# tier4/icp_rust

Measured on AMD Instinct MI355X. Metric: ICP iterations/sec on 1M-pt 3D pair, higher is better.
Workload: dtype f64

## Files before the change

### icp_rust_amd/csrc/gn_win.hip

```cpp
#include "common.hpp"
#include "gn_device.hpp"
#include "gn_win_device.hpp"
#include "gn_loop.hpp"

namespace icp {


template <bool SUMS, int BATCH = kWinBatch>
__device__ __forceinline__ void win_hist_body(const double2 *__restrict__ a, const double2 *__restrict__ b,
                                              const Pose &T, double *__restrict__ rx, double *__restrict__ ry,
                                              unsigned n, const WinParams &P, uint32_t *whist, WinState *st,
                                              GnScalars *scal, double *partials, int status_cls = -1) {
  __shared__ uint32_t lh[2 * kWinBins];
  if (SUMS && status_cls >= 0 && blockIdx.x == 0 && threadIdx.x < (unsigned)kShardStatusWords)
    whist[2 * kWinBins + threadIdx.x] = (int)threadIdx.x == status_cls ? 1u : 0u;
  double acc[SUMS ? kNSum : 1];
#pragma unroll
  for (int k = 0; k < (SUMS ? kNSum : 1); ++k) acc[k] = 0.;
#ifdef ICP_WIN_DEBUG
  long long wst[6];
  wst[0] = wall_clock64();
#endif
  for (unsigned i = threadIdx.x; i < 2u * kWinBins; i += kWinThreads) lh[i] = 0;
  __syncthreads();
// ... 662 lines not shown
  np.T = outer;
  if (usable) {
    double acc[kNAcc], delta[3];
#pragma unroll
    for (int k = 0; k < kNAcc; ++k) acc[k] = combine_sum(s_tot, k, sig);
    if (solve_update(acc, acc + 9, delta) &&
        !((delta[0] * delta[0] + delta[1] * delta[1]) + delta[2] * delta[2] < ICP_DELTA_NORM_THRESHOLD)) {
      bool in_range;
      const Pose step = transform_new_in_range(delta, &in_range);
      if (in_range) {
        const Pose inner = transform_mul(step, transform_identity());
        np.T = transform_mul(inner, outer);
        np.valid = 1;
      }
    }
  }
  *ahead = np;
  res->next_pose = np.T;
  res->next_valid = np.valid;
}

static_assert(kWinThreads == kReduceThreads, "the launches of an evaluation share the reduction tree's geometry");
template <bool LISTS>
__global__ __launch_bounds__(kWinThreads) void k_win_finish(const double *__restrict__ rx,
                                                            const double *__restrict__ ry, unsigned n, WinParams P,
                                                            uint32_t *whist, WinState *st, double *wmed, double *wring,
                                                            GnScalars *scal, const double *partials, int sum_blocks,
                                                            SelCtl *ctl, GnResult *res, unsigned seq,
                                                            const unsigned *__restrict__ llen, unsigned lcap,
                                                            AheadPose *ahead, Pose outer) {
  constexpr int PM = kWinCapMed / kReduceThreads, PR = kWinCapRing / kReduceThreads;
  WinSel sel;
#ifdef ICP_WIN_DEBUG
  long long fst[10];
  fst[0] = wall_clock64();
#endif
  double *const totals = const_cast<double *>(partials) + (size_t)kTreeMaxBlocks * (kNSum + 1);
  const bool fold_early = gridDim.x >= (unsigned)(kNSum + 1) && sum_blocks <= kReduceMaxBlocks;
  const double fold_x = (fold_early && blockIdx.x < (unsigned)(kNSum + 1)) ? fold_one_load(partials, sum_blocks, (int)blockIdx.x) : 0.;
  bool fail = win_compact_body<LISTS, true>(rx, ry, n, n, P, whist, st, wmed, wring, llen, lcap, sel);
  if (fold_early && blockIdx.x < (unsigned)(kNSum + 1)) {
    __shared__ double s_fold4[4];
    const double tot = fold_one_reduce(fold_x, sum_blocks, s_fold4);
    if (threadIdx.x == 0) __hip_atomic_store(&totals[blockIdx.x], tot, __ATOMIC_RELAXED, __HIP_MEMORY_SCOPE_AGENT);
  }
#ifdef ICP_WIN_DEBUG
  fst[1] = wall_clock64();
#endif
  if (!last_block_arrives(&ctl->t[2])) return;
#ifdef ICP_WIN_DEBUG
  fst[2] = wall_clock64();
#endif
  const unsigned tid = threadIdx.x;
  double med[2] = {0., 0.}, sig[2] = {0., 0.};
  __shared__ double s_tot[kNSum + 1];
  const int nan_flag = __hip_atomic_load(&scal->nan_flag, __ATOMIC_RELAXED, __HIP_MEMORY_SCOPE_AGENT);
  {
    double vm[2][PM], vr[2][PR];
#pragma unroll
    for (int d = 0; d < 2; ++d) {
#pragma unroll
      for (int u = 0; u < PM; ++u)
        vm[d][u] = (fail || tid + u * kReduceThreads < sel.med_cnt[d])
                       ? __hip_atomic_load(&wmed[(size_t)d * kWinCapMed + tid + u * kReduceThreads], __ATOMIC_RELAXED,
                                           __HIP_MEMORY_SCOPE_AGENT)
                       : 0.;
#pragma unroll
      for (int u = 0; u < PR; ++u)
        vr[d][u] = (fail || tid + u * kReduceThreads < sel.ring_cnt[d])
                       ? __hip_atomic_load(&wring[(size_t)d * kWinCapRing + tid + u * kReduceThreads], __ATOMIC_RELAXED,
                                           __HIP_MEMORY_SCOPE_AGENT)
                       : 0.;
    }
    unsigned got[4];
#pragma unroll
    for (int k = 0; k < 4; ++k)
      got[k] = __hip_atomic_load(&st->list_cnt[k][0], __ATOMIC_RELAXED, __HIP_MEMORY_SCOPE_AGENT);
    if (fold_early) {
      if (tid < kNSum + 1) s_tot[tid] = __hip_atomic_load(&totals[tid], __ATOMIC_RELAXED, __HIP_MEMORY_SCOPE_AGENT);
    } else if (sum_blocks <= kReduceMaxBlocks) {
      fold_block_sums_256(partials, sum_blocks, s_tot);
    } else {
      fold_block_sums_lean(partials, sum_blocks, s_tot);
    }
    for (unsigned i = tid; i < 2u * kWinBins; i += kWinThreads)
      __hip_atomic_store(&whist[i], 0u, __ATOMIC_RELAXED, __HIP_MEMORY_SCOPE_AGENT);
    fail = fail || got[0] != sel.med_cnt[0] || got[1] != sel.med_cnt[1] || got[2] != sel.ring_cnt[0] ||
           got[3] != sel.ring_cnt[1];
    const unsigned klo = (n - 1) / 2, khi = n / 2;
    if (!fail) {
      unsigned long long key[2][2];
      const double m_lo[2] = {sel.range[0][0], sel.range[1][0]}, m_hi[2] = {sel.range[0][1], sel.range[1][1]};
      const long long mlo[2] = {(long long)klo - sel.med_base[0], (long long)klo - sel.med_base[1]};
      const long long mhi[2] = {(long long)khi - sel.med_base[0], (long long)khi - sel.med_base[1]};
#ifdef ICP_WIN_DEBUG
      fst[3] = wall_clock64();
#endif
      select_n<2, PM>(vm, sel.med_cnt, m_lo, m_hi, mlo, mhi, key, fail);
#ifdef ICP_WIN_DEBUG
      fst[4] = wall_clock64();
#endif
      if (!fail) {
#pragma unroll
        for (int d = 0; d < 2; ++d) {
          med[d] = middle_of(n, key[d][0], key[d][1]);
#pragma unroll
          for (int u = 0; u < PR; ++u) vr[d][u] = fabs(vr[d][u] - med[d]);
        }
        const double r_lo[2] = {sel.range[0][2], sel.range[1][2]}, r_hi[2] = {sel.range[0][3], sel.range[1][3]};
        const long long dlo[2] = {(long long)klo - sel.inner[0], (long long)klo - sel.inner[1]};
        const long long dhi[2] = {(long long)khi - sel.inner[0], (long long)khi - sel.inner[1]};
        select_n<2, PR>(vr, sel.ring_cnt, r_lo, r_hi, dlo, dhi, key, fail);
        if (!fail) {
          sig[0] = ICP_PPF34 * middle_of(n, key[0][0], key[0][1]);
          sig[1] = ICP_PPF34 * middle_of(n, key[1][0], key[1][1]);
        } else {
          med[0] = med[1] = 0.;
        }
      }
    }
  }
  if (tid == 0 && fail) st->fail = 1u;
  asm volatile("s_waitcnt vmcnt(0)" ::: "memory");
  __syncthreads();
  if (ahead && tid == 0) fill_ahead_pose(s_tot, sig, !fail && !nan_flag, outer, ahead, res);
#ifdef ICP_WIN_DEBUG
  fst[5] = wall_clock64();
#endif
  publish_folded(s_tot, res, seq, sig, med, nan_flag, fail ? 2 : 0);
#ifdef ICP_WIN_DEBUG
  asm volatile("s_waitcnt vmcnt(0)" ::: "memory");
  fst[6] = wall_clock64();
  if (tid == 0 && seq % 16 == 5)
    printf("[F last blk %d of %d] compact %lld ticket %lld loads %lld sel1 %lld sel2 %lld publish %lld (x10ns) cnt %u %u %u %u\n", blockIdx.x,
           gridDim.x, fst[1] - fst[0], fst[2] - fst[1], fst[3] - fst[2], fst[4] - fst[3], fst[5] - fst[4], fst[6] - fst[5],
           sel.med_cnt[0], sel.med_cnt[1], sel.ring_cnt[0], sel.ring_cnt[1]);
#endif
}

struct PickLds {
  union {
    struct {
      uint32_t cum[2 * kWinBins];
      uint32_t med[2][kWinCapMed], ring[2][kWinCapRing];
    } g;
    SelectLds<2> sel;
  };
};

struct PickDimLds {
  union {
    struct {
      uint32_t cum[kWinBins];
      uint32_t med[kWinCapMed], ring[kWinCapRing];
    } g;
    SelectLds<1> sel;
  };
};

struct WinBins1 {
  unsigned mlo, mhi, a0, b1, i0, i1;
  bool fail;
};
struct WinSel1 {
  unsigned med_base, med_cnt, inner, ring_cnt;
  double range[4];
};

__device__ __forceinline__ WinBins1 win_resolve_dim(const uint32_t *__restrict__ row, unsigned n, const WinDim &w,
                                                    WinState *st, int d, uint32_t *cum, WinSel1 &sel) {
  __shared__ unsigned s_wtot[kReduceThreads / 64];
  __shared__ int s_j[2], s_t[2], s_rng[7];
  __shared__ unsigned s_selu[4];
  __shared__ double s_seld[4];
  constexpr int PER = kWinBins / kReduceThreads, NW = kReduceThreads / 64;
  static_assert(PER == 4, "one 16-byte load per thread");
  const int tid = threadIdx.x, lane = tid & 63, wave = tid >> 6;
  const unsigned klo = (n - 1) / 2, khi = n / 2;
  if (tid < 2) s_j[tid] = -1;
  const uint4 x = reinterpret_cast<const uint4 *>(row)[tid];
  const unsigned v[PER] = {x.x, x.y, x.z, x.w};
  const unsigned tot = (x.x + x.y) + (x.z + x.w);
  const unsigned inc = wave_scan_inclusive(tot);
  if (lane == 63) s_wtot[wave] = inc;
  __syncthreads();
  {
    unsigned wbase = 0;
#pragma unroll
    for (int q = 0; q < NW; ++q) wbase += (q < wave) ? s_wtot[q] : 0u;
    unsigned run = wbase + inc - tot;
#pragma unroll
    for (int i = 0; i < PER; ++i) {
      cum[PER * tid + i] = run;
      if (run <= klo && klo < run + v[i]) s_j[0] = PER * tid + i;
      if (run <= khi && khi < run + v[i]) s_j[1] = PER * tid + i;
      run += v[i];
    }
  }
  __syncthreads();
  WinGeom geo = {};
  if (wave < 2) {
    geo = window_geometry(cum, n, w, s_j[0], s_j[1]);
    const int t = geo.ok ? bracket_search(cum, n, w, geo, wave) : -1;
    if (lane == 0) s_t[wave] = t;
  }
  __syncthreads();
  if (wave == 0) {
    WinRanges R = {};
    unsigned med_base = 0, med_cnt = 0, inner = 0, ring_cnt = 0;
    double range[4] = {0., 0., 0., 0.};
    unsigned counted = 0;
#pragma unroll
    for (int q = 0; q < NW; ++q) counted += s_wtot[q];
    bool ok = counted == n && resolve_window(cum, n, w, geo, s_t[0], s_t[1], R, med_base, med_cnt, inner, ring_cnt, range);
    if (ok)
      ok = R.mlo >= kF1 && R.mhi < kC1 && R.i0 <= R.i1 && R.a0 >= kF0 && R.i0 - 1 < kC0 && R.i1 + 1 >= kF2 &&
           R.b1 <= kWinBins - 2;
    if (lane == 0) {
      s_rng[0] = R.mlo;
      s_rng[1] = R.mhi;
      s_rng[2] = R.a0;
      s_rng[3] = R.b1;
      s_rng[4] = R.i0;
      s_rng[5] = R.i1;
      s_rng[6] = ok ? 0 : 1;
      s_selu[0] = med_base;
      s_selu[1] = med_cnt;
      s_selu[2] = inner;
      s_selu[3] = ring_cnt;
#pragma unroll
      for (int k = 0; k < 4; ++k) s_seld[k] = range[k];
      if (st) {
        st->med_base[d] = med_base;
        st->med_cnt[d] = med_cnt;
        st->ring_inner[d] = inner;
        st->ring_cnt[d] = ring_cnt;
        st->med_lo[d] = range[0];
        st->med_hi[d] = range[1];
        st->ring_lo[d] = range[2];
        st->ring_hi[d] = range[3];
      }
    }
  }
  __syncthreads();
  WinBins1 B;
  B.mlo = (unsigned)s_rng[0];
  B.mhi = (unsigned)s_rng[1];
  B.a0 = (unsigned)s_rng[2];
  B.b1 = (unsigned)s_rng[3];
  B.i0 = (unsigned)s_rng[4];
  B.i1 = (unsigned)s_rng[5];
  B.fail = s_rng[6] != 0;
  sel.med_base = s_selu[0];
  sel.med_cnt = s_selu[1];
  sel.inner = s_selu[2];
  sel.ring_cnt = s_selu[3];
#pragma unroll
  for (int k = 0; k < 4; ++k) sel.range[k] = s_seld[k];
  return B;
}

struct PickArgs {
  unsigned n;
  WinParams P;
  uint32_t *whist;
  WinState *st;
  const double *seg_all;
  const unsigned short *dir_all;
  int segments;
  GnScalars *scal;
  const double *partials;
  int sum_blocks;
  GnResult *res;
  unsigned seq;
  AheadPose *ahead;
  Pose outer;
  WinJoin *join;
};

__device__ __forceinline__ void win_pick_dim_body(const PickArgs &A, const int d, const bool primary, PickDimLds &L) {
  const unsigned n = A.n;
  WinState *const st = A.st;
  const double *__restrict__ seg_all = A.seg_all;
  const unsigned short *__restrict__ dir_all = A.dir_all;
  WinJoin *const J = A.join;
  constexpr int PM = kWinCapMed / kReduceThreads, PR = kWinCapRing / kReduceThreads;
  static_assert(kReduceMaxBlocks * 2 == kReduceThreads, "two threads per segment");
  static_assert(kBktStage <= (1 << 12), "descriptor: segment << 12 | position");
  __shared__ double s_tot[kNSum + 1];
  __shared__ unsigned s_cnt[2];
  __shared__ int s_last;
  __shared__ unsigned s_pflags;
  __shared__ double s_pms[2];
  const unsigned tid = threadIdx.x;
#ifdef ICP_WIN_DEBUG
  long long pst[10];
  pst[0] = wall_clock64();
  for (int k = 1; k < 10; ++k) pst[k] = pst[0];
#define PSTAMP(k) pst[k] = wall_clock64()
#else
#define PSTAMP(k)
#endif
  if (tid < 2) s_cnt[tid] = 0;
  const int nan_flag = __hip_atomic_load(&A.scal->nan_flag, __ATOMIC_RELAXED, __HIP_MEMORY_SCOPE_AGENT);
  const unsigned stage_overflow = __hip_atomic_load(&st->stage_overflow, __ATOMIC_RELAXED, __HIP_MEMORY_SCOPE_AGENT);
  WinSel1 sel;
  const WinBins1 R = win_resolve_dim(A.whist + (size_t)d * kWinBins, n, A.P.d[d], primary ? st : nullptr, d, L.g.cum, sel);
  double fx[kFoldQ];
  fold256_half_load(A.partials, A.sum_blocks, d, fx);
  PSTAMP(1);
  const bool fail = R.fail;
  bool bucket_miss = stage_overflow != 0, sel_fail = false;
  double med = 0., sig = 0.;
  {
    const bool usable = !fail && !bucket_miss;
    const unsigned w = tid & (unsigned)(kReduceMaxBlocks - 1), part = tid / (unsigned)kReduceMaxBlocks;
    if (usable && (int)w < A.segments) {
      const unsigned short *dir = dir_all + (size_t)w * kBktDir;
      if (part == 0) {
        const unsigned fm = word_to_fine(d, R.mlo), len_m = R.mhi - R.mlo + 1u;
        const unsigned m0 = dir[fm], m_end = dir[fm + len_m];
        const unsigned cm = m_end - m0;
        if (cm) {
          const unsigned pos = atomicAdd(&s_cnt[0], cm);
          for (unsigned k = 0; k < cm; ++k)
            if (pos + k < (unsigned)kWinCapMed) L.g.med[pos + k] = (w << 12) | (m0 + k);
        }
      } else {
        const unsigned fa = word_to_fine(d, R.a0), fb = word_to_fine(d, R.i1 + 1u);
        const unsigned len_a = R.i0 - R.a0, len_b = R.b1 - R.i1;
        const unsigned a_beg = dir[fa], a_end = dir[fa + len_a], b_beg = dir[fb], b_end = dir[fb + len_b];
        const unsigned cr = (a_end - a_beg) + (b_end - b_beg);
        if (cr) {
          unsigned pos = atomicAdd(&s_cnt[1], cr);
          for (unsigned k = a_beg; k < a_end; ++k, ++pos)
            if (pos < (unsigned)kWinCapRing) L.g.ring[pos] = (w << 12) | k;
          for (unsigned k = b_beg; k < b_end; ++k, ++pos)
            if (pos < (unsigned)kWinCapRing) L.g.ring[pos] = (w << 12) | k;
        }
      }
    }
    __syncthreads();
    PSTAMP(2);
    if (usable) bucket_miss = s_cnt[0] != sel.med_cnt || s_cnt[1] != sel.ring_cnt;
    const bool go = usable && !bucket_miss;
    double vm[1][PM], vr[1][PR];
#pragma unroll
    for (int u = 0; u < PM; ++u) {
      const unsigned e = tid + u * kReduceThreads;
      vm[0][u] = 0.;
      if (go && e < sel.med_cnt) {
        const uint32_t x = L.g.med[e];
        vm[0][u] = seg_all[(size_t)(x >> 12) * kBktStage + (x & 0xfffu)];
      }
    }
#pragma unroll
    for (int u = 0; u < PR; ++u) {
      const unsigned e = tid + u * kReduceThreads;
      vr[0][u] = 0.;
      if (go && e < sel.ring_cnt) {
        const uint32_t x = L.g.ring[e];
        vr[0][u] = seg_all[(size_t)(x >> 12) * kBktStage + (x & 0xfffu)];
      }
    }
    {
      unsigned long long *row = reinterpret_cast<unsigned long long *>(A.whist + (size_t)d * kWinBins);
#pragma unroll
      for (int u = 0; u < kWinBins / 2 / kReduceThreads; ++u)
        __hip_atomic_store(&row[tid + u * kReduceThreads], 0ull, __ATOMIC_RELAXED, __HIP_MEMORY_SCOPE_AGENT);
    }
    fold256_half_reduce(fx, A.sum_blocks, s_tot + d * kFoldH);
    __syncthreads();
    PSTAMP(3);
    const unsigned klo = (n - 1) / 2, khi = n / 2;
    if (go) {
      unsigned long long key[1][2];
      const unsigned cm[1] = {sel.med_cnt}, cr[1] = {sel.ring_cnt};
      const double m_lo[1] = {sel.range[0]}, m_hi[1] = {sel.range[1]};
      const long long mlo[1] = {(long long)klo - sel.med_base}, mhi[1] = {(long long)khi - sel.med_base};
      select_n_lds<1, PM>(vm, cm, m_lo, m_hi, mlo, mhi, key, sel_fail, L.sel);
      PSTAMP(4);
      if (!sel_fail) {
        med = middle_of(n, key[0][0], key[0][1]);
#pragma unroll
        for (int u = 0; u < PR; ++u) vr[0][u] = fabs(vr[0][u] - med);
        const double r_lo[1] = {sel.range[2]}, r_hi[1] = {sel.range[3]};
        const long long dlo[1] = {(long long)klo - sel.inner}, dhi[1] = {(long long)khi - sel.inner};
        select_n_lds<1, PR>(vr, cr, r_lo, r_hi, dlo, dhi, key, sel_fail, L.sel);
        PSTAMP(5);
        if (!sel_fail) sig = ICP_PPF34 * middle_of(n, key[0][0], key[0][1]);
      }
    }
  }
  const unsigned flags = (fail ? 1u : 0u) | (bucket_miss ? 2u : 0u) | (sel_fail ? 4u : 0u);
  WinJoinDim *const mine = &J->dim[d];
  if (tid < (unsigned)kFoldH) __hip_atomic_store(&mine->tot[tid], s_tot[d * kFoldH + tid], __ATOMIC_RELAXED, __HIP_MEMORY_SCOPE_AGENT);
  if (tid == 64) {
    __hip_atomic_store(&mine->med, med, __ATOMIC_RELAXED, __HIP_MEMORY_SCOPE_AGENT);
    __hip_atomic_store(&mine->sig, sig, __ATOMIC_RELAXED, __HIP_MEMORY_SCOPE_AGENT);
    __hip_atomic_store(&mine->flags, flags, __ATOMIC_RELAXED, __HIP_MEMORY_SCOPE_AGENT);
  }
  asm volatile("s_waitcnt vmcnt(0)" ::: "memory");
  __syncthreads();
  PSTAMP(6);
  if (tid == 0)
    s_last = (int)(__hip_atomic_fetch_add(&J->ticket, 1u, __ATOMIC_RELAXED, __HIP_MEMORY_SCOPE_AGENT) & 1u);
  __syncthreads();
  if (!s_last) {
#ifdef ICP_WIN_DEBUG
    if (tid == 0 && A.seq % 16 == 5)
      printf("[P%d first] resolve %lld list %lld load+fold %lld sel1 %lld sel2 %lld store %lld (x10ns) cnt %u %u\n", d,
             pst[1] - pst[0], pst[2] - pst[1], pst[3] - pst[2], pst[4] - pst[3], pst[5] - pst[4], pst[6] - pst[5],
             sel.med_cnt, sel.ring_cnt);
#endif
    return;
  }
  const int o = 1 - d;
  const WinJoinDim *const other = &J->dim[o];
  static_assert(offsetof(WinJoinDim, tot) == 16 && offsetof(WinJoinDim, flags) == 96, "words of the record");
  if (tid < 13) {
    const unsigned long long x =
        __hip_atomic_load(reinterpret_cast<const unsigned long long *>(other) + tid, __ATOMIC_RELAXED, __HIP_MEMORY_SCOPE_AGENT);
    if (tid < 2) s_pms[tid] = __longlong_as_double((long long)x);
    else if (tid < 12) s_tot[o * kFoldH + (tid - 2)] = __longlong_as_double((long long)x);
    else s_pflags = (unsigned)x;
  }
  __syncthreads();
  PSTAMP(7);
  const unsigned all = flags | s_pflags;
  const bool any_fail = (all & 1u) != 0, any_bucket = (all & 2u) != 0;
  const bool failed = any_fail || (!any_bucket && (all & 4u) != 0);
  const bool missed = failed || any_bucket;
  const double m_me = missed ? 0. : med, s_me = missed ? 0. : sig, m_ot = missed ? 0. : s_pms[0], s_ot = missed ? 0. : s_pms[1];
  const double med2[2] = {d ? m_ot : m_me, d ? m_me : m_ot}, sig2[2] = {d ? s_ot : s_me, d ? s_me : s_ot};
  if (tid == 0) {
    if (missed) st->fail = 1u;
    else if (primary) st->fail = 0u;
    if (stage_overflow) __hip_atomic_store(&st->stage_overflow, 0u, __ATOMIC_RELAXED, __HIP_MEMORY_SCOPE_AGENT);
  }
  const int overflow = missed ? (failed ? 2 : 3) : 0;
  GnResult *const res = A.res;
  if (A.ahead) {
    if (tid == 0) fill_ahead_pose(s_tot, sig2, !missed && !nan_flag, A.outer, A.ahead, res);
    publish_values<1>(s_tot, res, sig2, med2, nan_flag, overflow);
    PSTAMP(8);
    __syncthreads();
    publish_seq(res, A.seq);
  } else {
    PSTAMP(8);
    publish_folded(s_tot, res, A.seq, sig2, med2, nan_flag, overflow);
  }
#ifdef ICP_WIN_DEBUG
  asm volatile("s_waitcnt vmcnt(0)" ::: "memory");
  PSTAMP(9);
  if (tid == 0 && A.seq % 16 == 5)
    printf("[P%d last] resolve %lld list %lld load+fold %lld sel1 %lld sel2 %lld store %lld ticket+loads %lld ahead %lld "
           "publish %lld (x10ns) cnt %u %u\n", d, pst[1] - pst[0], pst[2] - pst[1], pst[3] - pst[2], pst[4] - pst[3],
           pst[5] - pst[4], pst[6] - pst[5], pst[7] - pst[6], pst[8] - pst[7], pst[9] - pst[8], sel.med_cnt, sel.ring_cnt);
#endif
#undef PSTAMP
}

__global__ __launch_bounds__(kReduceThreads) void k_win_pick(PickArgs A) {
  __shared__ PickDimLds L;
  win_pick_dim_body(A, (int)blockIdx.x, true, L);
}

__global__ __launch_bounds__(kWinThreads, 4) void k_win_hist_sums_bkt2(HistBktArgs A, HistBktArgs B) {
  __shared__ HistBktLds S;
  const unsigned half = gridDim.x >> 1;
  if (blockIdx.x < half) win_hist_sums_bkt_body(A, blockIdx.x, half, S);
  else win_hist_sums_bkt_body(B, blockIdx.x - half, half, S);
}
__global__ __launch_bounds__(kReduceThreads) void k_win_pick2(PickArgs A, PickArgs B) {
  __shared__ PickDimLds L;
  if (blockIdx.x < 2u) win_pick_dim_body(A, (int)blockIdx.x, true, L);
  else win_pick_dim_body(B, (int)blockIdx.x - 2, false, L);
}

namespace {
constexpr long long kPipeTimeoutTicks = 300000000;
__device__ __forceinline__ void pst_u32(unsigned *p, unsigned v) { __hip_atomic_store(p, v, __ATOMIC_RELAXED, __HIP_MEMORY_SCOPE_SYSTEM); }
__device__ __forceinline__ void pst_f64(double *p, double v) { __hip_atomic_store(p, v, __ATOMIC_RELAXED, __HIP_MEMORY_SCOPE_SYSTEM); }
__device__ __forceinline__ unsigned pld_u32(const unsigned *p) { return __hip_atomic_load(p, __ATOMIC_RELAXED, __HIP_MEMORY_SCOPE_SYSTEM); }
__device__ __forceinline__ double pld_f64(const double *p) { return __hip_atomic_load(p, __ATOMIC_RELAXED, __HIP_MEMORY_SCOPE_SYSTEM); }

__device__ __forceinline__ bool pipe_poll(const unsigned long long *words, int count, unsigned gen, LoopInbox *const *box, int W,
                                          LoopInbox *me, unsigned *payload_or) {
  __shared__ int s_pok;
  __shared__ unsigned s_ppay;
  if (threadIdx.x < 64) {
    const int lane = (int)threadIdx.x;
    unsigned long long seen = 0;
    int ok = 1;
    const long long t0 = wall_clock64();
    for (;;) {
      bool here = true;
      if (lane < count) {
        seen = __hip_atomic_load(&words[lane], __ATOMIC_RELAXED, __HIP_MEMORY_SCOPE_SYSTEM);
        here = (int)((unsigned)seen - gen) >= 0;
      }
      if (__all(here)) break;
      int stop = 0;
      if (lane == 0) {
        if (pld_u32(&me->abort[0]) != 0u) stop = 1;
        else if (wall_clock64() - t0 > kPipeTimeoutTicks) {
          for (int q = 0; q < W; ++q) pst_u32(&box[q]->abort[0], 1u);
          stop = 1;
        }
      }
      if (__builtin_amdgcn_readfirstlane(stop)) {
        ok = 0;
        break;
      }
      __builtin_amdgcn_s_sleep(1);
    }
    unsigned pay = lane < count ? (unsigned)(seen >> 32) : 0u;
#pragma unroll
    for (int off = 32; off >= 1; off >>= 1) pay |= (unsigned)__shfl_xor((int)pay, off);
    if (lane == 0) {
      s_pok = ok;
      s_ppay = pay;
    }
  }
  __syncthreads();
  *payload_or = s_ppay;
  return s_pok != 0;
}
}

constexpr int kPipeFuse = 8;
struct PickRank {
  uint32_t *whist;
  WinState *st;
  const double *seg_all;
  const unsigned short *dir_all;
  GnScalars *scal;
  const double *partials;
  GnResult *res;
  AheadPose *ahead;
  int rank, b0, nbl;
  unsigned seq;
};
struct PickEval {
  unsigned n;
  unsigned gen;
  int ahead_on, pad;
  WinParams P;
  Pose outer;
  PickRank rk[kPipeFuse];
};
struct PickShardLaunch {
  int world, B, nranks, nevals;
  LoopInbox *inbox[kShardMaxWorld];
  PickEval ev[2];
};
static_assert(sizeof(PickShardLaunch) <= 4000, "kernel arguments");

__device__ __forceinline__ void win_pick_shard_body(const unsigned n, const unsigned gen, const bool ahead_on, const WinParams &P,
                                                    const Pose &outer, const PickRank &K, LoopInbox *const *box, const int W,
                                                    const int B, PickLds &L) {
  constexpr int PM = kWinCapMed / kReduceThreads, PR = kWinCapRing / kReduceThreads;
  constexpr int HW = 2 * kWinBins / kReduceThreads;
  __shared__ double s_tot[kNSum + 1];
  __shared__ unsigned s_cnt[4];
  __shared__ unsigned s_base[kShardMaxWorld + 1][4];
  __shared__ unsigned s_bad;
  const unsigned tid = threadIdx.x;
  const unsigned buf = gen & (unsigned)(kPipeBufs - 1);
  LoopInbox *const me = box[K.rank];
  PipeSlot *const mine = &me->pipe[buf];
  if (tid < 4) s_cnt[tid] = 0;
  if (tid == 0) s_bad = 0;
  const int nan_own = __hip_atomic_load(&K.scal->nan_flag, __ATOMIC_RELAXED, __HIP_MEMORY_SCOPE_AGENT);
  const unsigned ovf_own = __hip_atomic_load(&K.st->stage_overflow, __ATOMIC_RELAXED, __HIP_MEMORY_SCOPE_AGENT);
  {
    unsigned hv[HW];
#pragma unroll
    for (int k = 0; k < HW; ++k) hv[k] = __hip_atomic_load(&K.whist[tid + k * kReduceThreads], __ATOMIC_RELAXED, __HIP_MEMORY_SCOPE_AGENT);
    for (int q = 0; q < W; ++q) {
      uint32_t *dst = box[q]->pipe[buf].hist[K.rank];
#pragma unroll
      for (int k = 0; k < HW; ++k) pst_u32(&dst[tid + k * kReduceThreads], hv[k]);
    }
    const unsigned nrow = (unsigned)K.nbl * (unsigned)(kNSum + 1);
    for (unsigned j = tid; j < nrow; j += kReduceThreads) {
      const unsigned row = j / (unsigned)(kNSum + 1), k = j % (unsigned)(kNSum + 1);
      const double v = k < (unsigned)kNSum ? __hip_atomic_load(&K.partials[j], __ATOMIC_RELAXED, __HIP_MEMORY_SCOPE_AGENT) : 0.;
      for (int q = 0; q < W; ++q) pst_f64(&box[q]->pipe[buf].rows[(unsigned)K.b0 + row][k], v);
    }
#pragma unroll
    for (int k = 0; k < HW; ++k) __hip_atomic_store(&K.whist[tid + k * kReduceThreads], 0u, __ATOMIC_RELAXED, __HIP_MEMORY_SCOPE_AGENT);
    if (tid == 0 && ovf_own) __hip_atomic_store(&K.st->stage_overflow, 0u, __ATOMIC_RELAXED, __HIP_MEMORY_SCOPE_AGENT);
  }
  asm volatile("s_waitcnt vmcnt(0)" ::: "memory");
  __syncthreads();
  if ((int)tid < W) {
    const unsigned pay = (nan_own ? 1u : 0u) | (ovf_own ? 2u : 0u);
    __hip_atomic_store(&box[tid]->pipe[buf].flag_hist[K.rank], (unsigned long long)gen | ((unsigned long long)pay << 32), __ATOMIC_RELEASE,
                       __HIP_MEMORY_SCOPE_SYSTEM);
  }
  unsigned pay1 = 0;
  bool alive = pipe_poll(mine->flag_hist, W, gen, box, W, me, &pay1);
  const int nan_flag = (pay1 & 1u) ? 1 : 0;
  bool bucket_miss = (pay1 & 2u) != 0u;
  WinSel sel = {};
  WinBins R = {};
  R.fail = true;
  double fx[kFoldH];
#pragma unroll
  for (int k = 0; k < kFoldH; ++k) fx[k] = 0.;
  if (alive) {
    R = win_resolve<true, true, true>(&mine->hist[0][0], n, P, K.st, nullptr, 0u, L.g.cum, sel, W, (size_t)2 * kWinBins);
    if (B <= kReduceMaxBlocks) fold256_load<__HIP_MEMORY_SCOPE_SYSTEM>(&mine->rows[0][0], B, fx);
  }
  bool fail = R.fail;
  double med[2] = {0., 0.}, sig[2] = {0., 0.};
  {
    const unsigned w = tid & (unsigned)(kReduceMaxBlocks - 1), d = tid / (unsigned)kReduceMaxBlocks;
    const bool usable = alive && !fail && !bucket_miss;
    const unsigned mlo_d = d ? R.mlo[1] : R.mlo[0], mhi_d = d ? R.mhi[1] : R.mhi[0], a0_d = d ? R.a0[1] : R.a0[0];
    const unsigned b1_d = d ? R.b1[1] : R.b1[0], i0_d = d ? R.i0[1] : R.i0[0], i1_d = d ? R.i1[1] : R.i1[0];
    const unsigned len_m = usable ? mhi_d - mlo_d + 1u : 0u;
    const unsigned len_a = usable ? i0_d - a0_d : 0u, len_b = usable ? b1_d - i1_d : 0u;
    __syncthreads();
    if (usable && (int)w < K.nbl) {
      const unsigned short *dir = K.dir_all + (size_t)w * kBktDir;
      const unsigned fm = word_to_fine(d, mlo_d), fa = word_to_fine(d, a0_d), fb = word_to_fine(d, i1_d + 1u);
      const unsigned short q0 = dir[fm], q1 = dir[fm + len_m], q2 = dir[fa], q3 = dir[fa + len_a], q4 = dir[fb],
                           q5 = dir[fb + len_b];
// ... 235 lines not shown
#pragma unroll
    for (int d = 0; d < 2; ++d) {
#pragma unroll
      for (int u = 0; u < PM; ++u) pm[d][u] = where(d, tid + u * kReduceThreads);
#pragma unroll
      for (int u = 0; u < PR; ++u) pr[d][u] = where(2 + d, tid + u * kReduceThreads);
    }
    double vm[2][PM], vr[2][PR];
#pragma unroll
    for (int d = 0; d < 2; ++d) {
#pragma unroll
      for (int u = 0; u < PM; ++u) vm[d][u] = *pm[d][u];
#pragma unroll
      for (int u = 0; u < PR; ++u) vr[d][u] = *pr[d][u];
    }
    const unsigned klo = (n_total - 1) / 2, khi = n_total / 2;
    const unsigned em[2] = {got[0], got[1]}, er[2] = {got[2], got[3]};
    const double m_lo[2] = {st->med_lo[0], st->med_lo[1]}, m_hi[2] = {st->med_hi[0], st->med_hi[1]};
    const double r_lo[2] = {st->ring_lo[0], st->ring_lo[1]}, r_hi[2] = {st->ring_hi[0], st->ring_hi[1]};
    const long long mlo[2] = {(long long)klo - st->med_base[0], (long long)klo - st->med_base[1]};
    const long long mhi[2] = {(long long)khi - st->med_base[0], (long long)khi - st->med_base[1]};
    unsigned long long key[2][2];
#ifdef ICP_WIN_DEBUG
    sst[2] = wall_clock64();
#endif
    select_n<2, PM>(vm, em, m_lo, m_hi, mlo, mhi, key, fail);
#ifdef ICP_WIN_DEBUG
    sst[3] = wall_clock64();
#endif
    if (!fail) {
#pragma unroll
      for (int d = 0; d < 2; ++d) {
        med[d] = middle_of(n_total, key[d][0], key[d][1]);
#pragma unroll
        for (int u = 0; u < PR; ++u) vr[d][u] = fabs(vr[d][u] - med[d]);
      }
      const long long dlo[2] = {(long long)klo - st->ring_inner[0], (long long)klo - st->ring_inner[1]};
      const long long dhi[2] = {(long long)khi - st->ring_inner[0], (long long)khi - st->ring_inner[1]};
      select_n<2, PR>(vr, er, r_lo, r_hi, dlo, dhi, key, fail);
      if (!fail) {
        sig[0] = ICP_PPF34 * middle_of(n_total, key[0][0], key[0][1]);
        sig[1] = ICP_PPF34 * middle_of(n_total, key[1][0], key[1][1]);
      } else {
        med[0] = med[1] = 0.;
      }
    }
  }
  if (fail && h_counts && tid < 64)
    for (unsigned i = tid; i < 2u * kWinBins; i += 64) h_counts[i] = whist[i];
  __syncthreads();
  for (unsigned i = tid; i < 2u * kWinBins; i += kReduceThreads)
    __hip_atomic_store(&whist[i], 0u, __ATOMIC_RELAXED, __HIP_MEMORY_SCOPE_AGENT);
#ifdef ICP_WIN_DEBUG
  sst[4] = wall_clock64();
#endif
  asm volatile("s_waitcnt vmcnt(0)" ::: "memory");
  __syncthreads();
#ifdef ICP_WIN_DEBUG
  sst[5] = wall_clock64();
#endif
  publish_result(ordered, res, seq, sig, med, nan_flag, fail ? 2 : 0, blocks_total);
#ifdef ICP_WIN_DEBUG
  asm volatile("s_waitcnt vmcnt(0)" ::: "memory");
  sst[6] = wall_clock64();
  if (tid == 0 && seq % 16 == 3)
    printf("[SF] gather %lld fetch %lld sel1 %lld sel2+zero %lld drain %lld publish %lld (x10ns)\n", sst[1] - sst[0], sst[2] - sst[1],
           sst[3] - sst[2], sst[4] - sst[3], sst[5] - sst[4], sst[6] - sst[5]);
#endif
}

bool window_usable(const icp_handle *h, size_t n, WinParams *P, int kind, bool any_n, double f_override) {
  const Workspace &w = h->ws;
  if (n < kWinMinN || (n > kWinMaxN && !any_n)) return false;
  const bool own = Workspace::kind_has_slot(kind) && w.win_kind[kind].valid;
  if (!own && !w.win_valid) return false;
  const double *p_med = own ? w.win_kind[kind].med : w.win_med;
  const double *p_sigma = own ? w.win_kind[kind].sigma : w.win_sigma;
  double f = window_half_width(n, own ? w.win_kind[kind].wide : w.win_wide);
  if (f_override > 0.) f = f_override < 0.2 ? f_override : 0.2;
  return make_window(p_med, p_sigma, f, P);
}

double window_half_width(size_t n, bool wide) {
  if (n <= ((size_t)1 << 17)) return 0.2;
  constexpr double kHalfWidth = 0.05;
  double f = kHalfWidth * (wide ? 4. : 1.);
  if (n > 1000000) f *= 1e6 / (double)n;
  return f > 0.2 ? 0.2 : f;
}

bool make_window(const double med[2], const double sigma[2], double f, WinParams *P) { return make_window_hd(med, sigma, f, P); }

static unsigned tree_blocks(size_t n) {
  int blocks, threads;
  reduce_geometry(n, &blocks, &threads);
  return (unsigned)blocks;
}
bool bkt_fits(size_t n, const WinParams &P) { return tree_blocks(n) <= (unsigned)kReduceMaxBlocks && bkt_fits_rank(n, P); }
bool bkt_fits_rank(size_t n, const WinParams &P) {
  double frac = 0.;
  for (int d = 0; d < 2; ++d) {
    const WinDim &D = P.d[d];
    const double mad = 0.5 * ((D.x[4] + D.x[5]) - (D.x[2] + D.x[3]));
    frac += 1.04 * (D.x[1] - D.x[0]) / (ICP_PPF34 * mad);
  }
  return 2. * frac * ((double)n / tree_blocks(n)) <= (double)kBktStage;
}
static HistBktArgs bkt_hist_args(GnCtx &c, const double2 *a, const double2 *b, const Pose &T, unsigned n, const WinParams &P) {
  HistBktArgs A;
  A.a = a;
  A.b = b;
  A.T = T;
  A.n = n;
  A.P = P;
  A.whist = c.d_whist;
  A.st = c.d_wstate;
  A.scal = c.d_scal;
  A.partials = c.d_partials;
  A.seg_all = c.d_bkt;
  A.dir_all = c.d_bkt_dir;
  return A;
}
static PickArgs bkt_pick_args(GnCtx &c, unsigned n, const WinParams &P, bool ahead_on, const Pose &ahead_outer,
                              AheadPose *d_ahead = nullptr) {
  PickArgs A;
  A.n = n;
  A.P = P;
  A.whist = c.d_whist;
  A.st = c.d_wstate;
  A.seg_all = c.d_bkt;
  A.dir_all = c.d_bkt_dir;
  A.segments = (int)tree_blocks(n);
  A.scal = c.d_scal;
  A.partials = c.d_partials;
  A.sum_blocks = A.segments;
  A.res = c.h_res;
  A.seq = ++c.seq;
  A.ahead = ahead_on ? d_ahead : nullptr;
  A.outer = ahead_on ? ahead_outer : transform_identity();
  A.join = c.d_wjoin;
  return A;
}

hipError_t launch_bkt_pair(icp_handle *h, hipStream_t s, GnCtx &first, const double *a1, const double *b1, const WinParams &P1,
                           bool ahead_on, const Pose &ahead_outer, GnCtx &second, const double *a2, const double *b2,
                           const Pose &T2, const WinParams &P2, size_t n_) {
  Workspace &w = h->ws;
  const unsigned n = (unsigned)n_, blocks = tree_blocks(n_);
  if (blocks > (unsigned)kReduceMaxBlocks) return hipErrorInvalidValue;
  w.bkt_evals += 2;
  hipLaunchKernelGGL(k_win_hist_sums_bkt2, dim3(2 * blocks), dim3(kWinThreads), 0, s,
                     bkt_hist_args(first, (const double2 *)a1, (const double2 *)b1, transform_identity(), n, P1),
                     bkt_hist_args(second, (const double2 *)a2, (const double2 *)b2, T2, n, P2));
  hipLaunchKernelGGL(k_win_pick2, dim3(4), dim3(kReduceThreads), 0, s,
                     bkt_pick_args(first, n, P1, ahead_on, ahead_outer, w.d_ahead),
                     bkt_pick_args(second, n, P2, false, transform_identity()));
  second.bkt_pair_launched = true;
  return hipGetLastError();
}

hipError_t launch_shard_evals(const ShardPickRank *rk, int nranks, int world, int B, size_t n_total, unsigned gen0,
                              const ShardPickEval *ev, int nevals) {
  if (nranks < 1 || nranks > kPipeFuse || nevals < 1 || nevals > 2 || world < 1 || world > kShardMaxWorld || B < 1 || B > kTreeMaxBlocks)
    return hipErrorInvalidValue;
  for (int j = 0; j < nranks; ++j)
    if (rk[j].nbl < 1 || rk[j].nbl > kReduceMaxBlocks || rk[j].b0 < 0 || rk[j].b0 + rk[j].nbl > B || rk[j].rank < 0 || rk[j].rank >= world ||
        !rk[j].h->ws.d_loop_inbox)
      return hipErrorInvalidValue;
  PickShardLaunch L = {};
  L.world = world;
  L.B = B;
  L.nranks = nranks;
  L.nevals = nevals;
  const Workspace &w0 = rk[0].h->ws;
  for (int q = 0; q < kShardMaxWorld; ++q) L.inbox[q] = reinterpret_cast<LoopInbox *>(w0.loop_peers[q < world ? q : 0]);
  for (int j = 0; j < nranks; ++j) {
    icp_handle *h = rk[j].h;
    Workspace &w = h->ws;
    const unsigned nl = (unsigned)rk[j].n_local;
    GnCtx *ctx[2] = {nullptr, nullptr};
    HistBktArgs HA[2];
    for (int e = 0; e < nevals; ++e) {
      ctx[e] = ev[e].alt_ctx ? &w.alt : static_cast<GnCtx *>(&w);
      HA[e] = bkt_hist_args(*ctx[e], (const double2 *)rk[j].a[e], (const double2 *)rk[j].b[e], ev[e].T, nl, ev[e].P);
      PickRank &K = L.ev[e].rk[j];
      K.whist = ctx[e]->d_whist;
      K.st = ctx[e]->d_wstate;
      K.seg_all = ctx[e]->d_bkt;
      K.dir_all = ctx[e]->d_bkt_dir;
      K.scal = ctx[e]->d_scal;
      K.partials = ctx[e]->d_partials;
      K.res = ctx[e]->h_res;
      K.ahead = w.d_ahead;
      K.rank = rk[j].rank;
      K.b0 = rk[j].b0;
      K.nbl = rk[j].nbl;
      K.seq = ++ctx[e]->seq;
    }
    w.bkt_evals += (unsigned)nevals;
    if (nevals == 2)
      hipLaunchKernelGGL(k_win_hist_sums_bkt2, dim3(2u * (unsigned)rk[j].nbl), dim3(kWinThreads), 0, h->stream, HA[0], HA[1]);
    else
      hipLaunchKernelGGL(k_win_hist_sums_bkt, dim3((unsigned)rk[j].nbl), dim3(kWinThreads), 0, h->stream, HA[0]);
  }
  for (int e = 0; e < nevals; ++e) {
    L.ev[e].n = (unsigned)n_total;
    L.ev[e].gen = gen0 + (unsigned)e;
    L.ev[e].ahead_on = ev[e].ahead_on ? 1 : 0;
    L.ev[e].P = ev[e].P;
    L.ev[e].outer = ev[e].ahead_on ? ev[e].outer : transform_identity();
  }
  hipLaunchKernelGGL(k_win_pick_shard, dim3((unsigned)nevals, (unsigned)nranks), dim3(kReduceThreads), 0, rk[0].h->stream, L);
  return hipGetLastError();
}

hipError_t launch_weighted_gn_win(icp_handle *h, const double *d_a, const double *d_b, size_t n_, const Pose &T,
                                  const WinParams &P) {
  Workspace &w = h->ws;
  const unsigned n = (unsigned)n_;
  const unsigned per = kWinThreads * kWinBatch;
  unsigned hb = (n + per - 1) / per;
  if (hb > (unsigned)kWinBlocks) hb = kWinBlocks;
  const double2 *a = (const double2 *)d_a, *b = (const double2 *)d_b;
  hipStream_t s = h->stream;
  if (w.bkt_off > 0) --w.bkt_off;
  else if (bkt_fits(n_, P)) {
    ++w.bkt_evals;
    const HistBktArgs HA = bkt_hist_args(w, a, b, T, n, P);
    hipLaunchKernelGGL(k_win_hist_sums_bkt, dim3(tree_blocks(n_)), dim3(kWinThreads), 0, s, HA);
    hipLaunchKernelGGL(k_win_pick, dim3(2), dim3(kReduceThreads), 0, s, bkt_pick_args(w, n, P, w.ahead_on, w.ahead_outer, w.d_ahead));
    return hipGetLastError();
  }
  int blocks, threads;
  reduce_geometry(n_, &blocks, &threads);
  hipLaunchKernelGGL(k_win_hist_sums, dim3(blocks), dim3(threads), 0, s, a, b, T, w.d_rx, w.d_ry, n, P, w.d_whist,
                     w.d_wstate, w.d_scal, w.d_partials, -1);
  hipLaunchKernelGGL(k_win_finish<false>, dim3(hb), dim3(kWinThreads), 0, s, (const double *)w.d_rx,
                     (const double *)w.d_ry, n, P, w.d_whist, w.d_wstate, w.d_wmed, w.d_wring, w.d_scal,
                     (const double *)w.d_partials, blocks, w.d_ctl, w.h_res, ++w.seq, (const unsigned *)nullptr, 0u,
                     w.ahead_on ? w.d_ahead : (AheadPose *)nullptr, w.ahead_on ? w.ahead_outer : transform_identity());
  return hipGetLastError();
}

bool refine_applies(size_t n) {
  static const bool off = getenv("ICP_GN_NO_REFINE") != nullptr;
  return !off && n > kWinMaxN && n / kRefineSample >= 1 && n < 0xffffffffull;
}

hipError_t launch_sample_pairs(icp_handle *h, const double *d_a, const double *d_b, size_t n) {
  Workspace &w = h->ws;
  hipError_t e;
  if (!w.d_sa) {
    if ((e = hipMalloc(&w.d_sa, kRefineSample * 2 * sizeof(double))) != hipSuccess) return e;
    if ((e = hipMalloc(&w.d_sb, kRefineSample * 2 * sizeof(double))) != hipSuccess) return e;
    if ((e = hipHostMalloc(&w.h_whist, (size_t)2 * kWinBins * sizeof(uint32_t), hipHostMallocDefault)) != hipSuccess) return e;
    if ((e = hipMalloc(&w.d_rlist, 2 * kRefineListCap * sizeof(double))) != hipSuccess) return e;
    if ((e = hipMalloc(&w.d_rlist_len, 2 * sizeof(unsigned))) != hipSuccess) return e;
  }
  const unsigned stride = (unsigned)(n / kRefineSample);
  hipLaunchKernelGGL(k_sample_pairs, dim3((unsigned)(kRefineSample / 256)), dim3(256), 0, h->stream, (const double2 *)d_a,
                     (const double2 *)d_b, stride, (unsigned)kRefineSample, (double2 *)w.d_sa, (double2 *)w.d_sb);
  return hipGetLastError();
}

static unsigned win_hist_blocks(unsigned n) {
  const unsigned per = kWinThreads * kWinBatch;
  unsigned hb = (n + per - 1) / per;
  return hb > 4u * (unsigned)kWinBlocks ? 4u * (unsigned)kWinBlocks : hb;
}

hipError_t launch_win_first_pass(icp_handle *h, const double *d_a, const double *d_b, size_t n_, const Pose &T,
                                 const WinParams &P1) {
  Workspace &w = h->ws;
  const unsigned n = (unsigned)n_;
  int blocks, threads;
  reduce_geometry(n_, &blocks, &threads);
  hipLaunchKernelGGL(k_win_hist_sums_deep, dim3(blocks), dim3(threads), 0, h->stream, (const double2 *)d_a,
                     (const double2 *)d_b, T, w.d_rx, w.d_ry, n, P1, w.d_whist, w.d_wstate, w.d_scal, w.d_partials);
  hipError_t e = hipGetLastError();
  if (e != hipSuccess) return e;
  e = hipMemcpyAsync(w.h_whist, w.d_whist, (size_t)2 * kWinBins * sizeof(uint32_t), hipMemcpyDeviceToHost, h->stream);
  if (e != hipSuccess) return e;
  if ((e = hipMemsetAsync(w.d_rlist_len, 0, 2 * sizeof(unsigned), h->stream)) != hipSuccess) return e;
  return hipMemsetAsync(w.d_whist, 0, (size_t)2 * kWinBins * sizeof(uint32_t), h->stream);
}

static void bin_range(int j, const WinDim &w, double *lo, double *hi) {
  auto edge = [&](int k) -> double {
    if (k >= kWinBins - 1) return w.x[5];
    if (k >= kF2) return w.x[4] + (double)(k - kF2) / w.sf;
    if (k >= kC1) return w.x[3] + (double)(k - kC1) / w.sc;
    if (k >= kF1) return w.x[2] + (double)(k - kF1) / w.sf;
    if (k >= kC0) return w.x[1] + (double)(k - kC0) / w.sc;
    return w.x[0] + (double)(k - kF0) / w.sf;
  };
  *lo = edge(j);
  *hi = edge(j + 1);
}

bool refine_window(const uint32_t *hist, size_t n, const WinParams &P1, WinParams *P2) {
  double med[2], sigma[2];
  for (int d = 0; d < 2; ++d) {
    const uint32_t *c = hist + (size_t)d * kWinBins;
    const WinDim &w = P1.d[d];
    const size_t half = (n - 1) / 2;
    size_t run = 0;
    int jm = -1;
    for (int j = 0; j < kWinBins; ++j) {
      if (run + c[j] > half) {
// ... 57 lines not shown
```

Baseline: 10070.

## Gather pick candidates directly into LDS via wave scan instead of index lists

The pick kernel used to build per-segment descriptor lists in LDS through shared atomics, then issue a second dependent global gather from those descriptors. Each thread now loads up to twelve candidate values from its segment straight into registers before the barrier. It computes offsets with a wave-level inclusive scan plus a per-wave total table, and writes the values into double-typed LDS arrays, so the later select reads LDS only. This overlaps the global loads with the scan and removes the atomics and the second gather, at the cost of doubled LDS for the med/ring arrays and an extra barrier. The kernel also now takes a single struct argument and uses a branchless dispatch.

```diff
diff --git a/icp_rust_amd/csrc/gn_win.hip b/icp_rust_amd/csrc/gn_win.hip
--- a/icp_rust_amd/csrc/gn_win.hip
+++ b/icp_rust_amd/csrc/gn_win.hip
@@ -838,7 +838,7 @@
   union {
     struct {
       uint32_t cum[kWinBins];
-      uint32_t med[kWinCapMed], ring[kWinCapRing];
+      double med[kWinCapMed], ring[kWinCapRing];
     } g;
     SelectLds<1> sel;
   };
@@ -972,9 +972,8 @@
   WinJoin *const J = A.join;
   constexpr int PM = kWinCapMed / kReduceThreads, PR = kWinCapRing / kReduceThreads;
   static_assert(kReduceMaxBlocks * 2 == kReduceThreads, "two threads per segment");
-  static_assert(kBktStage <= (1 << 12), "descriptor: segment << 12 | position");
   __shared__ double s_tot[kNSum + 1];
-  __shared__ unsigned s_cnt[2];
+  __shared__ unsigned s_wcnt[kReduceThreads / 64];
   __shared__ int s_last;
   __shared__ unsigned s_pflags;
   __shared__ double s_pms[2];
@@ -987,7 +986,6 @@
 #else
 #define PSTAMP(k)
 #endif
-  if (tid < 2) s_cnt[tid] = 0;
   const int nan_flag = __hip_atomic_load(&A.scal->nan_flag, __ATOMIC_RELAXED, __HIP_MEMORY_SCOPE_AGENT);
   const unsigned stage_overflow = __hip_atomic_load(&st->stage_overflow, __ATOMIC_RELAXED, __HIP_MEMORY_SCOPE_AGENT);
   WinSel1 sel;
@@ -1000,54 +998,77 @@
   double med = 0., sig = 0.;
   {
     const bool usable = !fail && !bucket_miss;
+    constexpr int kPickU = 12;
     const unsigned w = tid & (unsigned)(kReduceMaxBlocks - 1), part = tid / (unsigned)kReduceMaxBlocks;
+    const unsigned lane = tid & 63u, wave = tid >> 6;
+    unsigned p0 = 0, l0 = 0, p1 = 0, l1 = 0;
     if (usable && (int)w < A.segments) {
       const unsigned short *dir = dir_all + (size_t)w * kBktDir;
       if (part == 0) {
         const unsigned fm = word_to_fine(d, R.mlo), len_m = R.mhi - R.mlo + 1u;
         const unsigned m0 = dir[fm], m_end = dir[fm + len_m];
-        const unsigned cm = m_end - m0;
-        if (cm) {
-          const unsigned pos = atomicAdd(&s_cnt[0], cm);
-          for (unsigned k = 0; k < cm; ++k)
-            if (pos + k < (unsigned)kWinCapMed) L.g.med[pos + k] = (w << 12) | (m0 + k);
-        }
+        p0 = m0;
+        l0 = m_end - m0;
       } else {
         const unsigned fa = word_to_fine(d, R.a0), fb = word_to_fine(d, R.i1 + 1u);
         const unsigned len_a = R.i0 - R.a0, len_b = R.b1 - R.i1;
         const unsigned a_beg = dir[fa], a_end = dir[fa + len_a], b_beg = dir[fb], b_end = dir[fb + len_b];
-        const unsigned cr = (a_end - a_beg) + (b_end - b_beg);
-        if (cr) {
-          unsigned pos = atomicAdd(&s_cnt[1], cr);
-          for (unsigned k = a_beg; k < a_end; ++k, ++pos)
-            if (pos < (unsigned)kWinCapRing) L.g.ring[pos] = (w << 12) | k;
-          for (unsigned k = b_beg; k < b_end; ++k, ++pos)
-            if (pos < (unsigned)kWinCapRing) L.g.ring[pos] = (w << 12) | k;
-        }
-      }
-    }
+        p0 = a_beg;
+        l0 = a_end - a_beg;
+        p1 = b_beg;
+        l1 = b_end - b_beg;
+      }
+    }
+    const unsigned cnt = l0 + l1;
+    const unsigned nld = cnt < (unsigned)kBktStage ? cnt : (unsigned)kBktStage;
+    const double *const seg = seg_all + (size_t)w * kBktStage;
+    auto member = [&](unsigned k) -> unsigned { return k < l0 ? p0 + k : p1 + (k - l0); };
+    double own[kPickU];
+#pragma unroll
+    for (int u = 0; u < kPickU; ++u) {
+      const unsigned at = member((unsigned)u);
+      own[u] = ((unsigned)u < nld && at < (unsigned)kBktStage) ? seg[at] : 0.;
+    }
+    const unsigned inc = wave_scan_inclusive(cnt);
+    if (lane == 63u) s_wcnt[wave] = inc;
     __syncthreads();
     PSTAMP(2);
-    if (usable) bucket_miss = s_cnt[0] != sel.med_cnt || s_cnt[1] != sel.ring_cnt;
+    unsigned before = 0, tot_m = 0, tot_r = 0;
+    {
+      constexpr unsigned HW = kReduceThreads / 64 / 2;
+#pragma unroll
+      for (unsigned q = 0; q < 2 * HW; ++q) {
+        const unsigned x = s_wcnt[q];
+        if (q < HW) tot_m += x;
+        else tot_r += x;
+        before += (q < wave && (q < HW) == (wave < HW)) ? x : 0u;
+      }
+    }
+    if (usable) bucket_miss = tot_m != sel.med_cnt || tot_r != sel.ring_cnt;
     const bool go = usable && !bucket_miss;
+    if (go) {
+      double *const vals = part ? L.g.ring : L.g.med;
+      const unsigned cap = part ? (unsigned)kWinCapRing : (unsigned)kWinCapMed;
+      const unsigned off = before + inc - cnt;
+#pragma unroll
+      for (int u = 0; u < kPickU; ++u)
+        if ((unsigned)u < nld && off + (unsigned)u < cap) vals[off + (unsigned)u] = own[u];
+      for (unsigned k = kPickU; k < nld; ++k) {
+        const unsigned at = member(k);
+        if (at < (unsigned)kBktStage && off + k < cap) vals[off + k] = seg[at];
+      }
+    }
+    __syncthreads();
     double vm[1][PM], vr[1][PR];
 #pragma unroll
     for (int u = 0; u < PM; ++u) {
       const unsigned e = tid + u * kReduceThreads;
-      vm[0][u] = 0.;
-      if (go && e < sel.med_cnt) {
-        const uint32_t x = L.g.med[e];
-        vm[0][u] = seg_all[(size_t)(x >> 12) * kBktStage + (x & 0xfffu)];
-      }
+      vm[0][u] = (go && e < sel.med_cnt) ? L.g.med[e] : 0.;
     }
 #pragma unroll
     for (int u = 0; u < PR; ++u) {
       const unsigned e = tid + u * kReduceThreads;
-      vr[0][u] = 0.;
-      if (go && e < sel.ring_cnt) {
-        const uint32_t x = L.g.ring[e];
-        vr[0][u] = seg_all[(size_t)(x >> 12) * kBktStage + (x & 0xfffu)];
-      }
+      vr[0][u] = (go && e < sel.ring_cnt) ? L.g.ring[e] : 0.;
     }
     {
       unsigned long long *row = reinterpret_cast<unsigned long long *>(A.whist + (size_t)d * kWinBins);
@@ -1095,7 +1116,7 @@
   if (!s_last) {
 #ifdef ICP_WIN_DEBUG
     if (tid == 0 && A.seq % 16 == 5)
-      printf("[P%d first] resolve %lld list %lld load+fold %lld sel1 %lld sel2 %lld store %lld (x10ns) cnt %u %u\n", d,
+      printf("[P%d first] resolve %lld dir+scan %lld place+fold %lld sel1 %lld sel2 %lld store %lld (x10ns) cnt %u %u\n", d,
              pst[1] - pst[0], pst[2] - pst[1], pst[3] - pst[2], pst[4] - pst[3], pst[5] - pst[4], pst[6] - pst[5],
              sel.med_cnt, sel.ring_cnt);
 #endif
@@ -1140,7 +1161,7 @@
   asm volatile("s_waitcnt vmcnt(0)" ::: "memory");
   PSTAMP(9);
   if (tid == 0 && A.seq % 16 == 5)
-    printf("[P%d last] resolve %lld list %lld load+fold %lld sel1 %lld sel2 %lld store %lld ticket+loads %lld ahead %lld "
+    printf("[P%d last] resolve %lld dir+scan %lld place+fold %lld sel1 %lld sel2 %lld store %lld ticket+loads %lld ahead %lld "
            "publish %lld (x10ns) cnt %u %u\n", d, pst[1] - pst[0], pst[2] - pst[1], pst[3] - pst[2], pst[4] - pst[3],
            pst[5] - pst[4], pst[6] - pst[5], pst[7] - pst[6], pst[8] - pst[7], pst[9] - pst[8], sel.med_cnt, sel.ring_cnt);
 #endif
@@ -1158,10 +1179,13 @@
   if (blockIdx.x < half) win_hist_sums_bkt_body(A, blockIdx.x, half, S);
   else win_hist_sums_bkt_body(B, blockIdx.x - half, half, S);
 }
-__global__ __launch_bounds__(kReduceThreads) void k_win_pick2(PickArgs A, PickArgs B) {
+struct PickPairArgs {
+  PickArgs e[2];
+};
+__global__ __launch_bounds__(kReduceThreads) void k_win_pick2(PickPairArgs X) {
   __shared__ PickDimLds L;
-  if (blockIdx.x < 2u) win_pick_dim_body(A, (int)blockIdx.x, true, L);
-  else win_pick_dim_body(B, (int)blockIdx.x - 2, false, L);
+  const unsigned second = blockIdx.x >> 1;
+  win_pick_dim_body(X.e[second], (int)(blockIdx.x & 1u), second == 0u, L);
 }
 
 namespace {
@@ -1703,9 +1727,10 @@
   hipLaunchKernelGGL(k_win_hist_sums_bkt2, dim3(2 * blocks), dim3(kWinThreads), 0, s,
                      bkt_hist_args(first, (const double2 *)a1, (const double2 *)b1, transform_identity(), n, P1),
                      bkt_hist_args(second, (const double2 *)a2, (const double2 *)b2, T2, n, P2));
-  hipLaunchKernelGGL(k_win_pick2, dim3(4), dim3(kReduceThreads), 0, s,
-                     bkt_pick_args(first, n, P1, ahead_on, ahead_outer, w.d_ahead),
-                     bkt_pick_args(second, n, P2, false, transform_identity()));
+  PickPairArgs X;
+  X.e[0] = bkt_pick_args(first, n, P1, ahead_on, ahead_outer, w.d_ahead);
+  X.e[1] = bkt_pick_args(second, n, P2, false, transform_identity());
+  hipLaunchKernelGGL(k_win_pick2, dim3(4), dim3(kReduceThreads), 0, s, X);
   second.bkt_pair_launched = true;
   return hipGetLastError();
 }
```

Result: faster. 10380, median of 6 (+3.1%).
